# DeepLearnPhysics/dynamic-gcnn

Hardware: AMD Instinct MI355X
Metric: point-clouds/sec fwd+bwd at (B,N,k,C)=(24,2048,20,3), 1/2/4/8 MI355X (higher is better)
Workload: dtype f32

## Files before the change

### dynamic-gcnn_amd/csrc/knn.hip

```cpp
#include "knn_common.h"
#include <type_traits>
#include <stdlib.h>

namespace {

constexpr int ROWS = 64;
constexpr int WAVES = 4;
constexpr int TJ = 128;
constexpr int PERW = TJ / WAVES;

constexpr int SQ_ROWS = 64;
__global__ __launch_bounds__(256) void sqnorm_kernel(const float* __restrict__ x, int64_t ldx, int64_t rows, int C,
                                                     float* __restrict__ sq) {
  extern __shared__ float sq_tile[];
  const int64_t r0 = (int64_t)blockIdx.x * SQ_ROWS;
  const int t = threadIdx.x;
  const int S = C + 1;
  for (int e = t; e < SQ_ROWS * C; e += 256) {
    const int rr = e / C, cc = e - rr * C;
    if (r0 + rr < rows) sq_tile[rr * S + cc] = x[(r0 + rr) * ldx + cc];
  }
  __syncthreads();
  if (t < SQ_ROWS && r0 + t < rows) {
    float s = 0.0f;
// ... 1035 lines not shown
        qn = 0;
      }
    }
  }
  if (qn > 0) process(qn, 0, (nt - 1) & 1);
  __syncthreads();
  if (tid < ROWS && row0 + tid < N) cnt[grow0 + tid] = cnt_s[tid];
}

__global__ __launch_bounds__(256) void knn_select_kernel(const unsigned long long* __restrict__ ent, const int* __restrict__ cnt,
                                                         int64_t rows, int cap, int k, int32_t* __restrict__ idx) {
  const int lane = threadIdx.x & 63;
  const int64_t row = (int64_t)blockIdx.x * 4 + (threadIdx.x >> 6);
  if (row >= rows) return;
  const int S = cnt[row];
  const unsigned long long* buf = ent + row * cap;
  int32_t* out = idx + row * k;
  if (S <= 64) {
    unsigned long long key = (lane < S) ? buf[lane] : ~0ull;
    key = wave_sort64(key, lane);
    if (lane < k) out[lane] = (int32_t)(unsigned)key;
    return;
  }
  unsigned long long key[KA_MAXE];
#pragma unroll
  for (int q = 0; q < KA_MAXE; ++q) {
    const int e = lane + 64 * q;
    key[q] = (e < S) ? buf[e] : ~0ull;
  }
  const unsigned long long best = wave_lowest64<KA_MAXE>(key, S, lane);
  if (lane < k) out[lane] = (int32_t)(unsigned)best;
}

int g_knn_bf16f = -1;
int knn_bf16f_mode() {
  if (g_knn_bf16f < 0) {
    const char* e = getenv("DGCNN_KNN_BF16F");
    g_knn_bf16f = e ? ((e[0] == 'a') ? 2 : atoi(e)) : 2;
  }
  return g_knn_bf16f;
}

int g_knn_valu = 0;
bool knn_force_valu() { return g_knn_valu == 1; }

template <int LP, int MAXSTEPS, class Clouds = DenseClouds>
__global__ __launch_bounds__(256) void knn_seed_bound_kernel(const float* __restrict__ x, const float* __restrict__ sq, Clouds cl,
                                                             int64_t ldx, const int32_t* __restrict__ seed, int64_t ldseed, int k,
                                                             int64_t rows, float* __restrict__ tau0) {
  constexpr int PPS = 64 / LP;
  constexpr int RW = 2;
  const int lane = threadIdx.x & 63;
  const int64_t per = ((rows + 7) / 8 + 4 * RW - 1) / (4 * RW) * (4 * RW);
  const int64_t g0 = (int64_t)(blockIdx.x & 7) * per + ((int64_t)(blockIdx.x >> 3) * 4 + (threadIdx.x >> 6)) * RW;
  if (g0 >= rows || ((int64_t)(blockIdx.x >> 3) * 4 + (threadIdx.x >> 6)) * RW >= per) return;
  const int slot = lane / LP, cq = lane % LP;
  const int steps = (k + PPS - 1) / PPS;
  int jj[RW], nn[RW];
  int64_t gr[RW];
  const float* xc[RW];
  const float* sc[RW];
#pragma unroll
  for (int w = 0; w < RW; ++w) {
    gr[w] = (g0 + w < rows) ? g0 + w : rows - 1;
    jj[w] = (lane < k) ? seed[gr[w] * ldseed + lane] : -1 - lane;
    if constexpr (Clouds::kPacked) {
// ... 118 lines not shown
int dispatch_k(const float* x, const float* sq, int B, int N, int C, int64_t ldx, int k, int vec_ok,
               int32_t* idx, const float* tau0, hipStream_t st) {
  if (k <= 8) launch_knn<CP, 8>(x, sq, B, N, C, ldx, k, vec_ok, idx, tau0, st);
  else if (k <= 20) launch_knn<CP, 20>(x, sq, B, N, C, ldx, k, vec_ok, idx, tau0, st);
  else if (k <= 40) launch_knn<CP, 40>(x, sq, B, N, C, ldx, k, vec_ok, idx, tau0, st);
  else launch_knn<CP, 64>(x, sq, B, N, C, ldx, k, vec_ok, idx, tau0, st);
  return dg::check_launch("dgcnn_knn_f32");
}

}

extern "C" int dgcnn_knn_force_valu(int on) {
  const int prev = knn_force_valu() ? 1 : 0;
  g_knn_valu = on ? 1 : 0;
  return prev;
}

extern "C" int dgcnn_knn_bf16_filter(int mode) {
  const int prev = knn_bf16f_mode();
  g_knn_bf16f = mode;
  return prev;
}

namespace dg {
size_t knn_grid_workspace_bytes(int B, int N);
bool knn_grid_applicable(int C, int k);
int knn_grid_min_n();
int launch_knn_grid(const float* x, const float* sq, int B, int N, int C, int64_t ldx, int k, int32_t* idx, void* ws, hipStream_t st);
size_t knn_grid_seg_workspace_bytes(int rows, int nseg);
int launch_knn_grid_seg(const float* x, const float* sq, int nseg, const int32_t* seg_off, int rows, int max_n, int C, int64_t ldx, int k,
                        int32_t* idx, void* ws, hipStream_t st);
}

static size_t knn_sq_bytes(int B, int N) { return (((size_t)B * (size_t)N * sizeof(float)) + 255) & ~(size_t)255; }
static bool knn_append_lx(int N) { return N < 8192; }
static int knn_append_cap(int k, int N) {
  if (knn_append_lx(N)) return k <= 20 ? 256 : (k <= 40 ? 384 : 512);
  return k <= 20 ? 320 : (k <= 40 ? 448 : 512);
}
static bool knn_append_shape(int C, int k) { return C > 16 && C <= 64 && C % 4 == 0 && k <= 64; }
static size_t knn_append_rows_bytes(size_t rows, int cap) {
  return ((rows * sizeof(int) + 255) & ~(size_t)255) + rows * (size_t)cap * sizeof(unsigned long long);
}
static size_t knn_append_bytes(int B, int N, int k) { return knn_append_rows_bytes((size_t)B * (size_t)N, knn_append_cap(k, N)); }
static int knn_append_tighten_mask(bool lx) {
  static int tight = -1;
  if (tight < 0) { const char* e = getenv("DGCNN_KNN_TIGHTEN_EVERY"); tight = e ? atoi(e) : 0; if (tight < 0 || (tight & (tight - 1))) tight = 1; }
  return (tight ? tight : (lx ? 4 : 8)) - 1;
}

extern "C" int64_t dgcnn_knn_workspace_bytes(int B, int N, int C, int k) {
  if (B <= 0 || N <= 0) return 0;
  size_t n = 2 * knn_sq_bytes(B, N);
  if (dg::knn_grid_applicable(C, k)) n += dg::knn_grid_workspace_bytes(B, N);
  else if (knn_append_shape(C, k)) n += knn_append_bytes(B, N, k);
  return (int64_t)n;
}

static int g_knn_seed_min_n = -2;
static int knn_seed_min_n() {
  if (g_knn_seed_min_n == -2) {
    const char* e = getenv("DGCNN_KNN_SEED_MIN_N");
    g_knn_seed_min_n = e ? atoi(e) : -1;
  }
  return g_knn_seed_min_n;
}
extern "C" int dgcnn_knn_seed_min_n(int n) {
  const int prev = knn_seed_min_n();
  if (n >= -1) g_knn_seed_min_n = n;
  return prev;
}

static int g_knn_append = -1;
static bool knn_append_on() {
  if (g_knn_append < 0) {
    const char* e = getenv("DGCNN_KNN_APPEND");
    g_knn_append = e ? atoi(e) : 1;
  }
  return g_knn_append != 0;
}
extern "C" int dgcnn_knn_append(int on) {
  const int prev = knn_append_on() ? 1 : 0;
  if (on >= 0) g_knn_append = on ? 1 : 0;
  return prev;
}

static int g_knn_npr[2] = {-1, -1};
static int knn_append_products(bool lx) {
  if (g_knn_npr[0] < 0) {
    int a = 1, b = 1;
    const char* e = getenv("DGCNN_KNN_APPEND_NPR");
    if (e) sscanf(e, "%d,%d", &a, &b);
    g_knn_npr[0] = (a == 3) ? 3 : 1;
    g_knn_npr[1] = (b == 3) ? 3 : 1;
  }
  return g_knn_npr[lx ? 0 : 1];
}
extern "C" int dgcnn_knn_append_products(int n) {
  const int prev = knn_append_products(true);
  if (n == 1 || n == 3) g_knn_npr[0] = g_knn_npr[1] = n;
  return prev;
}

static int g_knn_hist = -1;
static int knn_hist_stride(int N) {
  if (g_knn_hist < 0) {
    const char* e = getenv("DGCNN_KNN_HIST");
    g_knn_hist = e ? atoi(e) : 2;
    if (g_knn_hist != 0 && g_knn_hist != 1 && g_knn_hist != 2 && g_knn_hist != 4) g_knn_hist = 2;
  }
  return N >= 256 ? g_knn_hist : 0;
}
extern "C" int dgcnn_knn_hist(int stride) {
  const int prev = knn_hist_stride(1 << 20);
  if (stride == 0 || stride == 1 || stride == 2 || stride == 4) g_knn_hist = stride;
  return prev;
}

static int knn_impl(const char* what, const float* x, int B, int N, int C, int64_t ldx, int k, const int32_t* seed, int64_t ldseed,
                    int kseed, int32_t* idx, void* ws, size_t ws_bytes, void* stream) {
  DG_REQUIRE(x && idx && ws, DGCNN_EINVAL, "%s: null pointer", what);
  DG_REQUIRE(B > 0 && N > 0 && C > 0 && ldx >= C, DGCNN_EINVAL, "%s: bad shape B=%d N=%d C=%d", what, B, N, C);
  DG_REQUIRE(k > 0 && k <= N, DGCNN_EINVAL, "%s: k=%d must be in [1, N=%d] (tf.nn.top_k raises otherwise)", what, k, N);
  DG_REQUIRE(k <= 64, DGCNN_EUNSUP, "%s: k=%d > 64 unsupported", what, k);
  DG_REQUIRE(C <= 128, DGCNN_EUNSUP, "%s: C=%d > 128 unsupported", what, C);
  DG_REQUIRE((reinterpret_cast<uintptr_t>(ws) & 15) == 0 && ws_bytes >= knn_sq_bytes(B, N), DGCNN_EINVAL,
             "%s: workspace must be 16-byte aligned and hold dgcnn_knn_workspace_bytes(B, N, C, k) bytes (got %zu)", what, ws_bytes);
  hipStream_t st = (hipStream_t)stream;
  float* sq_ws = reinterpret_cast<float*>(ws);
  const int64_t rows = (int64_t)B * N;
  const int vec_ok = (ldx % 4 == 0) && ((reinterpret_cast<uintptr_t>(x) & 15) == 0);
  const size_t grid_off = 2 * knn_sq_bytes(B, N);
  const bool append = knn_append_on() && knn_append_shape(C, k) && vec_ok && !knn_force_valu() && knn_bf16f_mode() != 0 &&
                      ws_bytes >= grid_off + knn_append_bytes(B, N, k);
  const int min_n = knn_seed_min_n() >= 0 ? knn_seed_min_n() : (append ? 0 : 4096);
  const bool seeded = seed && kseed >= k && kseed <= 64 && C > 4 && C <= 64 && C % 4 == 0 && vec_ok && !knn_force_valu() &&
                      N >= min_n && (int64_t)N * ldx < ((int64_t)1 << 31) && ws_bytes >= 2 * knn_sq_bytes(B, N);
  const bool grid_ws = dg::knn_grid_applicable(C, k) && !knn_force_valu() && ws_bytes >= grid_off + dg::knn_grid_workspace_bytes(B, N);
  dg::launch(sqnorm_kernel, dim3((unsigned)dg::cdiv(rows, SQ_ROWS)), dim3(256), sizeof(float) * SQ_ROWS * (C + 1), st, x,
                     ldx, rows, C, sq_ws);
  if (grid_ws && N >= dg::knn_grid_min_n())
    return dg::launch_knn_grid(x, sq_ws, B, N, C, ldx, k, idx, reinterpret_cast<char*>(ws) + grid_off, st);
  float* tau0 = nullptr;
  if (seeded) {
    tau0 = reinterpret_cast<float*>(reinterpret_cast<char*>(ws) + knn_sq_bytes(B, N));
    if (!launch_seed_bound(x, sq_ws, rows, DenseClouds(N), C, ldx, seed, ldseed, k, tau0, st)) tau0 = nullptr;
  }
  if (tau0 && append) {
    char* base = reinterpret_cast<char*>(ws) + grid_off;
    int* cnt = reinterpret_cast<int*>(base);
    unsigned long long* ent = reinterpret_cast<unsigned long long*>(base + (((size_t)rows * sizeof(int) + 255) & ~(size_t)255));
    const int cap = knn_append_cap(k, N);
    const dim3 grid((unsigned)dg::cdiv(N, ROWS), (unsigned)B);
    const int npr = knn_append_products(knn_append_lx(N));
    const int tmask = knn_append_tighten_mask(knn_append_lx(N));
#define DG_KA(LXV, NPRV) dg::launch((knn_bf16a_kernel<LXV, NPRV>), grid, dim3(256), 0, st, x, (const float*)sq_ws, N, C, ldx, k, (const float*)tau0, cap, ent, cnt, tmask)
    if (knn_append_lx(N)) { if (npr == 1) DG_KA(true, 1); else DG_KA(true, 3); }
    else { if (npr == 1) DG_KA(false, 1); else DG_KA(false, 3); }
#undef DG_KA
    dg::launch(knn_select_kernel, dim3((unsigned)dg::cdiv(rows, 4)), dim3(256), 0, st, (const unsigned long long*)ent, (const int*)cnt, rows,
               cap, k, idx);
    return dg::check_launch(what);
  }
  if (C <= 4) {
    const int hs = knn_hist_stride(N);
    if (hs > 0 && !knn_force_valu() && k <= 64 && N >= 4 * k * hs && ws_bytes >= 2 * knn_sq_bytes(B, N)) {
      float* tb = reinterpret_cast<float*>(reinterpret_cast<char*>(ws) + knn_sq_bytes(B, N));
      const dim3 hg((unsigned)dg::cdiv(N, 64), (unsigned)B);
      if (hs == 1) dg::launch(knn_hist_bound_kernel<1>, hg, dim3(256), 0, st, x, (const float*)sq_ws, N, C, ldx, k, tb);
      else if (hs == 2) dg::launch(knn_hist_bound_kernel<2>, hg, dim3(256), 0, st, x, (const float*)sq_ws, N, C, ldx, k, tb);
      else dg::launch(knn_hist_bound_kernel<4>, hg, dim3(256), 0, st, x, (const float*)sq_ws, N, C, ldx, k, tb);
      tau0 = tb;
    }
    return dispatch_k<4>(x, sq_ws, B, N, C, ldx, k, vec_ok, idx, tau0, st);
  }
  if (C <= 16) return dispatch_k<16>(x, sq_ws, B, N, C, ldx, k, vec_ok, idx, tau0, st);
  if (C <= 64) return dispatch_k<64>(x, sq_ws, B, N, C, ldx, k, vec_ok, idx, tau0, st);
  return dispatch_k<128>(x, sq_ws, B, N, C, ldx, k, vec_ok, idx, tau0, st);
}

extern "C" int dgcnn_knn_f32(const float* x, int B, int N, int C, int64_t ldx, int k, int32_t* idx,
                             void* ws, size_t ws_bytes, void* stream) {
  return knn_impl("dgcnn_knn_f32", x, B, N, C, ldx, k, nullptr, 0, 0, idx, ws, ws_bytes, stream);
}

extern "C" int dgcnn_knn_seeded_f32(const float* x, int B, int N, int C, int64_t ldx, int k, const int32_t* seed, int64_t ldseed,
                                    int kseed, int32_t* idx, void* ws, size_t ws_bytes, void* stream) {
  DG_REQUIRE(!seed || (ldseed >= kseed && kseed > 0), DGCNN_EINVAL, "dgcnn_knn_seeded_f32: bad seed shape");
  return knn_impl("dgcnn_knn_seeded_f32", x, B, N, C, ldx, k, seed, ldseed, kseed, idx, ws, ws_bytes, stream);
}

extern "C" int64_t dgcnn_knn_seg_workspace_bytes(int rows, int max_n, int C, int k) {
  if (rows <= 0 || max_n <= 0) return 0;
  size_t n = 2 * knn_sq_bytes(1, rows);
  if (knn_append_shape(C, k)) n += knn_append_rows_bytes((size_t)rows, knn_append_cap(k, max_n));
  return (int64_t)n;
}

extern "C" int dgcnn_knn_seg_f32(const float* x, int64_t ldx, int C, int k, int nseg, const int32_t* seg_off, int rows, int min_n,
                                 int max_n, const int32_t* seed, int64_t ldseed, int kseed, int32_t* idx, void* ws, size_t ws_bytes,
                                 void* stream) {
  const char* what = "dgcnn_knn_seg_f32";
  DG_REQUIRE(x && idx && ws && seg_off, DGCNN_EINVAL, "%s: null pointer", what);
  DG_REQUIRE(nseg > 0 && nseg <= 65535 && rows > 0 && C > 0 && ldx >= C, DGCNN_EINVAL, "%s: bad shape nseg=%d rows=%d C=%d", what,
             nseg, rows, C);
// ... 16 lines not shown
  const size_t aux = 2 * knn_sq_bytes(1, rows);
  const bool lx = knn_append_lx(max_n);
  const int cap = knn_append_cap(k, max_n);
  const bool append = knn_append_on() && knn_append_shape(C, k) && vec_ok && !knn_force_valu() && knn_bf16f_mode() != 0 &&
                      ws_bytes >= aux + knn_append_rows_bytes((size_t)rows, cap);
  const int seed_min = knn_seed_min_n() >= 0 ? knn_seed_min_n() : 0;
  const bool seeded = append && seed && kseed >= k && kseed <= 64 && min_n >= seed_min && (int64_t)max_n * ldx < ((int64_t)1 << 31);
  dg::launch(sqnorm_kernel, dim3((unsigned)dg::cdiv(rows, SQ_ROWS)), dim3(256), sizeof(float) * SQ_ROWS * (C + 1), st, x, ldx,
             (int64_t)rows, C, sq_ws);
  if (seeded && launch_seed_bound(x, sq_ws, (int64_t)rows, cl, C, ldx, seed, ldseed, k, tb, st)) {
    char* base = reinterpret_cast<char*>(ws) + aux;
    int* cnt = reinterpret_cast<int*>(base);
    unsigned long long* ent = reinterpret_cast<unsigned long long*>(base + (((size_t)rows * sizeof(int) + 255) & ~(size_t)255));
    const dim3 grid((unsigned)dg::cdiv(max_n, ROWS), (unsigned)nseg);
    const int npr = knn_append_products(lx);
    const int tmask = knn_append_tighten_mask(lx);
#define DG_KA(LXV, NPRV) dg::launch((knn_bf16a_kernel<LXV, NPRV, PackedClouds>), grid, dim3(256), 0, st, x, (const float*)sq_ws, cl, C, ldx, k, (const float*)tb, cap, ent, cnt, tmask)
    if (lx) { if (npr == 1) DG_KA(true, 1); else DG_KA(true, 3); }
    else { if (npr == 1) DG_KA(false, 1); else DG_KA(false, 3); }
#undef DG_KA
    dg::launch(knn_select_kernel, dim3((unsigned)dg::cdiv(rows, 4)), dim3(256), 0, st, (const unsigned long long*)ent, (const int*)cnt,
               (int64_t)rows, cap, k, idx);
    return dg::check_launch(what);
  }
  if (C <= 4) {
    const int hs = knn_hist_stride(min_n);
    const float* tau0 = nullptr;
    if (hs > 0 && !knn_force_valu() && min_n >= 4 * k * hs && tb_ok) {
      const dim3 hg((unsigned)dg::cdiv(max_n, 64), (unsigned)nseg);
      if (hs == 1) dg::launch(knn_hist_bound_kernel<1, PackedClouds>, hg, dim3(256), 0, st, x, (const float*)sq_ws, cl, C, ldx, k, tb);
      else if (hs == 2) dg::launch(knn_hist_bound_kernel<2, PackedClouds>, hg, dim3(256), 0, st, x, (const float*)sq_ws, cl, C, ldx, k, tb);
      else dg::launch(knn_hist_bound_kernel<4, PackedClouds>, hg, dim3(256), 0, st, x, (const float*)sq_ws, cl, C, ldx, k, tb);
      tau0 = tb;
    }
    return dispatch_k_packed<4>(x, sq_ws, cl, max_n, C, ldx, k, vec_ok, idx, tau0, st);
  }
  if (C <= 16) return dispatch_k_packed<16>(x, sq_ws, cl, max_n, C, ldx, k, vec_ok, idx, nullptr, st);
  if (C <= 64) return dispatch_k_packed<64>(x, sq_ws, cl, max_n, C, ldx, k, vec_ok, idx, nullptr, st);
  return dispatch_k_packed<128>(x, sq_ws, cl, max_n, C, ldx, k, vec_ok, idx, nullptr, st);
}

extern "C" int64_t dgcnn_knn_seg_grid_workspace_bytes(int rows, int nseg) {
  if (rows <= 0 || nseg <= 0) return 0;
  return (int64_t)(knn_sq_bytes(1, rows) + dg::knn_grid_seg_workspace_bytes(rows, nseg));
}

extern "C" int dgcnn_knn_seg_grid_f32(const float* x, int64_t ldx, int C, int k, int nseg, const int32_t* seg_off, int rows, int min_n,
                                      int max_n, int32_t* idx, void* ws, size_t ws_bytes, void* stream) {
  const char* what = "dgcnn_knn_seg_grid_f32";
  DG_REQUIRE(x && idx && ws && seg_off, DGCNN_EINVAL, "%s: null pointer", what);
  DG_REQUIRE(nseg > 0 && nseg <= 65535 && rows > 0 && C > 0 && ldx >= C, DGCNN_EINVAL, "%s: bad shape nseg=%d rows=%d C=%d", what,
             nseg, rows, C);
  DG_REQUIRE(C <= 4 && k <= 40, DGCNN_EINVAL, "%s: C=%d k=%d: the cell grid searches raw coordinates (C <= 4) for k <= 40", what, C, k);
  DG_REQUIRE(min_n > 0 && min_n <= max_n && max_n <= rows && (int64_t)min_n * nseg <= rows && (int64_t)max_n * nseg >= rows,
             DGCNN_EINVAL, "%s: cloud sizes min_n=%d max_n=%d do not fit %d rows in %d clouds", what, min_n, max_n, rows, nseg);
  DG_REQUIRE(k > 0 && k <= min_n, DGCNN_EINVAL, "%s: k=%d must be in [1, smallest cloud=%d] (tf.nn.top_k raises otherwise)", what, k,
             min_n);
  DG_REQUIRE((reinterpret_cast<uintptr_t>(ws) & 15) == 0 && ws_bytes >= (size_t)dgcnn_knn_seg_grid_workspace_bytes(rows, nseg),
             DGCNN_EINVAL, "%s: workspace must be 16-byte aligned and hold dgcnn_knn_seg_grid_workspace_bytes(rows, nseg) bytes (got %zu)",
             what, ws_bytes);
  hipStream_t st = (hipStream_t)stream;
  float* sq_ws = reinterpret_cast<float*>(ws);
  dg::launch(sqnorm_kernel, dim3((unsigned)dg::cdiv(rows, SQ_ROWS)), dim3(256), sizeof(float) * SQ_ROWS * (C + 1), st, x, ldx,
             (int64_t)rows, C, sq_ws);
  return dg::launch_knn_grid_seg(x, sq_ws, nseg, seg_off, rows, max_n, C, ldx, k, idx, reinterpret_cast<char*>(ws) + knn_sq_bytes(1, rows),
                                 st);
// ... 2 lines not shown
```

### dynamic-gcnn_amd/dgcnn/_engine.py

```python
from __future__ import annotations

import contextlib
import os
from collections import OrderedDict

import numpy as np
import torch

from . import _hip as H
from . import _planes as PL

BN_EPS = 1e-3
DROPOUT_KEEP = 0.7
WS_BYTES = 256 << 20
EDGE_MLP_LITERAL = False
EDGE_MATERIALIZE_Y = False
WGRAD_SIDE_STREAM = os.environ.get("DGCNN_SIDE_STREAM", "1") != "0"
EDGE_BWD_FUSED_L0 = True
FUSE_DROPOUT = True
BF16_FUSED_BWD = True
EDGE_BWD_REDUCE_POINTS = True
SIDE_STREAM_MIN_ROWS = 16384
SIDE_STREAM_LOW_PRIORITY = os.environ.get("DGCNN_SIDE_LOW_PRIORITY", "0") not in ("0", "")
SIDE_STREAM_RESERVE_CUS = int(os.environ.get("DGCNN_SIDE_RESERVE_CUS", "0"))
# ... 405 lines not shown
        self.min_n, self.max_n = int(sizes.min()), int(sizes.max())
        self._dev = None
        self._rg = None

    def check_k(self, k):
        if k <= 0 or k > self.min_n:
            raise ValueError("k_nn: k=%d must be in [1, smallest cloud=%d] (tf.nn.top_k raises otherwise)" % (k, self.min_n))

    def device(self, dev):
        if self._dev is None or self._dev.device != dev:
            self._dev = torch.from_numpy(self.host.astype(np.int32)).to(dev)
        return self._dev

    def row_group(self, dev):
        if self._rg is None or self._rg.device != dev:
            rg = np.repeat(np.arange(self.nseg, dtype=np.int32), np.diff(self.host))
            self._rg = torch.from_numpy(rg).to(dev)
        return self._rg


def knn(x2d, B, N, k, seed=None, seg=None):
    if seg is not None:
        return knn_packed(x2d, k, seg, seed=seed)
    C = x2d.shape[1]
    idx = torch.empty((B, N, k), dtype=torch.int32, device=x2d.device)
    nws = int(H.load().dgcnn_knn_workspace_bytes(B, N, C, k))
    ws = torch.empty((nws,), dtype=torch.uint8, device=x2d.device)
    Cp, kc = (4 if C <= 4 else 16 if C <= 16 else 64 if C <= 64 else 128), (8 if k <= 8 else 20 if k <= 20 else 40 if k <= 40 else 64)
    seeded = (KNN_SEED and seed is not None and seed.dim() == 3 and seed.shape[0] == B and seed.shape[1] == N and seed.shape[2] >= k
              and seed.dtype == torch.int32 and seed.is_contiguous())
    if seeded and 16 < C <= 64:
        tag = "knn_call<C%d,k%d>[sqnorm_kernel+knn_seed_bound_kernel+knn_bf16a_kernel+knn_select_kernel]" % (Cp, kc)
    elif C <= 4:
        tag = "knn_call<C%d,k%d>[%s]" % (Cp, kc, "knn_grid_*" if N >= 4096 else "sqnorm_kernel+knn_hist_bound_kernel+knn_kernel")
    else:
        tag = "knn_call<C%d,k%d>[sqnorm_kernel+%s]" % (Cp, kc, "knn_bf16f_kernel" if N >= 8192 else "knn_mfma_kernel")
    if (KNN_SEED and seed is not None and seed.dim() == 3 and seed.shape[0] == B and seed.shape[1] == N and seed.shape[2] >= k and
            seed.dtype == torch.int32 and seed.is_contiguous()):
        H.call("dgcnn_knn_seeded_f32", x2d.data_ptr(), B, N, C, H.ld2(x2d), k, seed.data_ptr(), int(seed.shape[2]), int(seed.shape[2]),
               idx.data_ptr(), ws.data_ptr(), nws, tag=tag, work=2.0 * B * N * N * C)
    else:
        H.call("dgcnn_knn_f32", x2d.data_ptr(), B, N, C, H.ld2(x2d), k, idx.data_ptr(), ws.data_ptr(), nws, tag=tag,
               work=2.0 * B * N * N * C)
    return idx


def knn_packed(x2d, k, seg, seed=None):
    R, C = x2d.shape
    if R != seg.rows:
        raise ValueError("offsets end at %d, the tower has %d rows" % (seg.rows, R))
    seg.check_k(k)
    off = seg.device(x2d.device)
    idx = torch.empty((1, R, k), dtype=torch.int32, device=x2d.device)
    n = seg.host[1:] - seg.host[:-1]
    Cp, kc = (4 if C <= 4 else 16 if C <= 16 else 64 if C <= 64 else 128), (8 if k <= 8 else 20 if k <= 20 else 40 if k <= 40 else 64)
    if C <= 4 and H.load().dgcnn_knn_seg_grid_use(C, k, seg.nseg, R, seg.min_n, seg.max_n, int((n * n).sum())):
        nws = int(H.load().dgcnn_knn_seg_grid_workspace_bytes(R, seg.nseg))
        ws = torch.empty((nws,), dtype=torch.uint8, device=x2d.device)
        H.call("dgcnn_knn_seg_grid_f32", x2d.data_ptr(), H.ld2(x2d), C, k, seg.nseg, off.data_ptr(), R, seg.min_n, seg.max_n,
               idx.data_ptr(), ws.data_ptr(), nws, tag="knn_seg_call<C4,k%d>[sqnorm_kernel+knn_grid_*]" % kc,
               work=2.0 * float((n * n).sum()) * C)
        return idx
    nws = int(H.load().dgcnn_knn_seg_workspace_bytes(R, seg.max_n, C, k))
    ws = torch.empty((nws,), dtype=torch.uint8, device=x2d.device)
    seeded = (KNN_SEED and seed is not None and seed.dim() == 3 and seed.shape[0] == 1 and seed.shape[1] == R and seed.shape[2] >= k
              and seed.dtype == torch.int32 and seed.is_contiguous())
    if seeded and 16 < C <= 64:
# ... 811 lines not shown
```

### dynamic-gcnn_amd/dgcnn/_hip.py

```python
from __future__ import annotations

import ctypes
import os

import torch

_HERE = os.path.dirname(os.path.abspath(__file__))
LIB_PATH = os.environ.get("DGCNN_HIP_LIB") or os.path.join(_HERE, "libdgcnn_hip.so")
STAT_SLOTS = 32

c_int, c_i64, c_f32, c_f64, c_vp, c_sz, c_u64 = (ctypes.c_int, ctypes.c_int64, ctypes.c_float, ctypes.c_double,
                                                  ctypes.c_void_p, ctypes.c_size_t, ctypes.c_uint64)

PROTOTYPES = {
    "dgcnn_version": [],
    "dgcnn_last_error": [],
    "dgcnn_knn_workspace_bytes": [c_int, c_int, c_int, c_int],
    "dgcnn_knn_grid": [c_int],
    "dgcnn_knn_force_valu": [c_int],
    "dgcnn_knn_bf16_filter": [c_int],
    "dgcnn_knn_f32": [c_vp, c_int, c_int, c_int, c_i64, c_int, c_vp, c_vp, c_sz, c_vp],
    "dgcnn_knn_seed_min_n": [c_int],
    "dgcnn_knn_append": [c_int],
    "dgcnn_knn_append_products": [c_int],
    "dgcnn_knn_hist": [c_int],
    "dgcnn_knn_seeded_f32": [c_vp, c_int, c_int, c_int, c_i64, c_int, c_vp, c_i64, c_int, c_vp, c_vp, c_sz, c_vp],
    "dgcnn_knn_seg_workspace_bytes": [c_int, c_int, c_int, c_int],
    "dgcnn_knn_seg_f32": [c_vp, c_i64, c_int, c_int, c_int, c_vp, c_int, c_int, c_int, c_vp, c_i64, c_int, c_vp, c_vp, c_sz, c_vp],
    "dgcnn_knn_seg_grid_workspace_bytes": [c_int, c_int],
    "dgcnn_knn_seg_grid_f32": [c_vp, c_i64, c_int, c_int, c_int, c_vp, c_int, c_int, c_int, c_vp, c_vp, c_sz, c_vp],
    "dgcnn_knn_seg_grid_use": [c_int, c_int, c_int, c_int, c_int, c_int, c_i64],
    "dgcnn_edge_gather_f32": [c_vp, c_i64, c_vp, c_int, c_int, c_int, c_int, c_vp, c_vp],
    "dgcnn_edge_gather_bwd_f32": [c_vp, c_vp, c_int, c_int, c_int, c_int, c_vp, c_i64, c_vp],
    "dgcnn_edge_mlp_f32": [c_vp, c_i64, c_vp, c_vp, c_int, c_int, c_int, c_int, c_int, c_vp, c_vp, c_vp],
    "dgcnn_edge_mlp_wgrad_f32": [c_vp, c_i64, c_vp, c_vp, c_int, c_int, c_int, c_int, c_int, c_vp, c_f32,
                                 c_vp, c_sz, c_vp],
    "dgcnn_edge_mlp_dgrad_scatter_f32": [c_vp, c_vp, c_vp, c_int, c_int, c_int, c_int, c_int, c_vp, c_i64, c_vp],
    "dgcnn_edge_nbr_gemm_f32": [c_vp, c_i64, c_vp, c_vp, c_vp, c_i64, c_int, c_int, c_int, c_int, c_int, c_vp, c_vp, c_vp],
    "dgcnn_edge_nbr_wgrad_f32": [c_vp, c_i64, c_vp, c_vp, c_int, c_int, c_int, c_int, c_int, c_vp, c_f32,
                                 c_vp, c_sz, c_vp],
    "dgcnn_edge_csr_build": [c_vp, c_int, c_int, c_int, c_vp, c_vp, c_vp, c_vp],
    "dgcnn_edge_gather_sum_f32": [c_vp, c_vp, c_vp, c_i64, c_int, c_vp, c_i64, c_vp],
    "dgcnn_edge_weight_split_f32": [c_vp, c_int, c_int, c_vp, c_vp],
    "dgcnn_edge_gather_add_f32": [c_vp, c_i64, c_vp, c_i64, c_vp, c_int, c_int, c_int, c_int, c_vp, c_vp, c_vp],
    "dgcnn_edge_wgrad_combine_f32": [c_vp, c_int, c_int, c_vp, c_vp],
    "dgcnn_edge_bn_act_kreduce_f32": [c_vp, c_i64, c_vp, c_i64, c_vp, c_int, c_int, c_int, c_int, c_vp, c_vp, c_vp,
                                      c_int, c_vp, c_i64, c_vp, c_i64, c_vp, c_vp],
    "dgcnn_edge_bn_bwd_reduce_f32": [c_vp, c_i64, c_vp, c_i64, c_vp, c_int, c_int, c_int, c_int, c_vp, c_vp, c_vp,
                                     c_int, c_vp, c_i64, c_vp, c_i64, c_vp, c_i64, c_vp, c_vp, c_vp],
    "dgcnn_edge_bn_bwd_reduce_points_f32": [c_vp, c_i64, c_vp, c_i64, c_vp, c_vp, c_i64, c_vp, c_i64, c_vp, c_i64, c_int,
                                            c_int, c_vp, c_vp],
    "dgcnn_edge_bn_bwd_apply_f32": [c_vp, c_i64, c_vp, c_i64, c_vp, c_int, c_int, c_int, c_int, c_vp, c_vp, c_vp,
                                    c_int, c_vp, c_i64, c_vp, c_i64, c_vp, c_i64, c_vp, c_vp, c_vp, c_vp, c_i64, c_vp,
                                    c_f32, c_vp],
    "dgcnn_edge_bn_bwd_apply_wgrad_f32": [c_vp, c_i64, c_vp, c_i64, c_vp, c_int, c_int, c_int, c_int, c_vp, c_vp, c_vp,
                                          c_vp, c_i64, c_vp, c_i64, c_vp, c_i64, c_vp, c_vp, c_vp, c_i64, c_int, c_vp, c_vp, c_f32,
                                          c_vp, c_sz, c_vp],
    "dgcnn_bn1_act_dropout_f32": [c_vp, c_i64, c_int, c_vp, c_vp, c_vp, c_int, c_f32, c_vp, c_vp, c_i64, c_vp],
# ... 53 lines not shown
    "dgcnn_adam_f32": [c_vp, c_vp, c_vp, c_vp, c_i64, c_f32, c_f32, c_f32, c_f32, c_vp],
    "dgcnn_edge_mlp_bf16_supported": [c_int, c_int, c_int],
    "dgcnn_round_bf16_f32": [c_vp, c_vp, c_i64, c_vp],
    "dgcnn_edge_mlp_bf16": [c_vp, c_i64, c_vp, c_vp, c_int, c_int, c_int, c_int, c_int, c_vp, c_vp],
    "dgcnn_edge_mlp_bf16_stats": [c_vp, c_i64, c_vp, c_vp, c_int, c_int, c_int, c_int, c_int, c_vp, c_vp],
    "dgcnn_edge_mlp_bf16_bn_kreduce": [c_vp, c_i64, c_vp, c_vp, c_int, c_int, c_int, c_int, c_int, c_vp, c_vp, c_vp, c_vp, c_i64,
                                       c_vp, c_i64, c_vp, c_int, c_vp],
    "dgcnn_edge_mlp_bf16_bwd_supported": [c_int, c_int, c_int],
    "dgcnn_edge_mlp_bf16_bwd_workspace_bytes": [c_int, c_int, c_int, c_int, c_int],
    "dgcnn_edge_mlp_bf16_bwd": [c_vp, c_i64, c_vp, c_vp, c_int, c_int, c_int, c_int, c_int, c_vp, c_vp, c_vp, c_vp, c_i64, c_vp,
                                c_vp, c_i64, c_vp, c_i64, c_vp, c_vp, c_vp, c_i64, c_vp, c_vp, c_f32, c_vp, ctypes.c_size_t, c_vp],
    "dgcnn_edge_gather_sum_bf16": [c_vp, c_vp, c_vp, c_i64, c_int, c_vp, c_i64, c_vp],
    "dgcnn_plan_begin": [],
    "dgcnn_plan_end": [c_vp],
    "dgcnn_plan_abort": [],
    "dgcnn_plan_replay": [c_vp],
    "dgcnn_plan_info": [c_vp, c_vp, c_vp, c_vp, c_vp],
    "dgcnn_plan_destroy": [c_vp],
    "dgcnn_stream_wait": [c_vp, c_vp],
    "dgcnn_stream_create": [c_int, c_int, c_vp],
    "dgcnn_stream_destroy": [c_vp],
    "dgcnn_stream_priority_range": [c_vp, c_vp],
    "dgcnn_memset_async": [c_vp, c_int, c_sz, c_vp],
    "dgcnn_comm_available": [],
    "dgcnn_comm_unique_id": [c_vp],
    "dgcnn_comm_init": [c_int, c_int, c_vp, c_vp],
    "dgcnn_comm_destroy": [c_vp],
    "dgcnn_comm_info": [c_vp, c_vp, c_vp, c_vp],
    "dgcnn_allreduce_f32": [c_vp, c_i64, c_vp, c_vp],
    "dgcnn_broadcast_f32": [c_vp, c_i64, c_int, c_vp, c_vp],
    "dgcnn_comm_counters": [c_vp, c_vp],
}

INT64_RESULTS = ("dgcnn_knn_workspace_bytes", "dgcnn_knn_seg_workspace_bytes", "dgcnn_knn_seg_grid_workspace_bytes",
                 "dgcnn_edge_mlp_bf16_bwd_workspace_bytes", "dgcnn_seg_colsum_workspace_bytes")

_lib = None


class HipError(RuntimeError):
    pass


def load():
    global _lib
    if _lib is None:
        if not os.path.exists(LIB_PATH):
            raise HipError("libdgcnn_hip.so not built (%s); run `python -c 'import __graft_entry__ as g; g.build()'` "
                           "or `make -C dynamic-gcnn_amd/csrc` -- there is no CPU fallback" % LIB_PATH)
        lib = ctypes.CDLL(LIB_PATH)
        for name, args in PROTOTYPES.items():
            fn = getattr(lib, name)
            fn.argtypes = args
            fn.restype = (ctypes.c_char_p if name == "dgcnn_last_error" else
                          ctypes.c_int64 if name in INT64_RESULTS else ctypes.c_int)
        _lib = lib
    return _lib


def set_gemm_arith(mode):
    lib = load()
    if lib.dgcnn_gemm_set_arith(int(mode)) != 0:
        raise ValueError(lib.dgcnn_last_error().decode())


def set_stat_slots(n):
    global STAT_SLOTS
# ... 160 lines not shown
```

### include/dgcnn_hip.h

```cpp
#ifndef DGCNN_HIP_H_
#define DGCNN_HIP_H_

#include <stddef.h>
#include <stdint.h>

#ifdef __cplusplus
extern "C" {
#endif

#define DGCNN_OK 0
#define DGCNN_EINVAL (-1)
#define DGCNN_ELAUNCH (-2)
#define DGCNN_ENOSPC (-3)
#define DGCNN_EUNSUP (-4)

#define DGCNN_STAT_SLOTS 32
int dgcnn_set_stat_slots(int n);
int dgcnn_get_stat_slots(void);

int dgcnn_version(void);
const char* dgcnn_last_error(void);

int64_t dgcnn_knn_workspace_bytes(int B, int N, int C, int k);
int dgcnn_knn_grid(int mode);
int dgcnn_knn_force_valu(int on);
int dgcnn_knn_bf16_filter(int mode);
int dgcnn_knn_f32(const float* x, int B, int N, int C, int64_t ldx, int k, int32_t* idx,
                  void* ws, size_t ws_bytes, void* stream);
int dgcnn_knn_seeded_f32(const float* x, int B, int N, int C, int64_t ldx, int k, const int32_t* seed, int64_t ldseed,
                         int kseed, int32_t* idx, void* ws, size_t ws_bytes, void* stream);
int dgcnn_knn_seed_min_n(int n);
int dgcnn_knn_append(int on);
int dgcnn_knn_append_products(int n);
int dgcnn_knn_hist(int stride);
int64_t dgcnn_knn_seg_workspace_bytes(int rows, int max_n, int C, int k);
int dgcnn_knn_seg_f32(const float* x, int64_t ldx, int C, int k, int nseg, const int32_t* seg_off, int rows, int min_n, int max_n,
                      const int32_t* seed, int64_t ldseed, int kseed, int32_t* idx, void* ws, size_t ws_bytes, void* stream);
int64_t dgcnn_knn_seg_grid_workspace_bytes(int rows, int nseg);
int dgcnn_knn_seg_grid_f32(const float* x, int64_t ldx, int C, int k, int nseg, const int32_t* seg_off, int rows, int min_n, int max_n,
                           int32_t* idx, void* ws, size_t ws_bytes, void* stream);
int dgcnn_knn_seg_grid_use(int C, int k, int nseg, int rows, int min_n, int max_n, int64_t sum_n2);

int dgcnn_edge_mlp_bf16_supported(int C, int k, int F);
int dgcnn_edge_mlp_bf16_bwd_supported(int C, int k, int F);
int64_t dgcnn_edge_mlp_bf16_bwd_workspace_bytes(int B, int N, int C, int k, int F);
int dgcnn_edge_mlp_bf16_bwd(const float* x, int64_t ldx, const int32_t* idx, const float* W0, int B, int N, int C, int k, int F,
                            const float* mean, const float* rstd, const float* beta, const float* mx, int64_t ldmx,
                            const float* cnt, const float* dmx, int64_t lddmx, const float* dmn, int64_t lddmn, double* red,
                            void* dYb, float* dysum, int64_t lddysum, float* dW0, float* dbeta, float dbeta_beta, void* ws,
                            size_t ws_bytes, void* stream);
int dgcnn_edge_gather_sum_bf16(const void* dY, const int32_t* off, const int32_t* rev, int64_t R, int F, float* S, int64_t lds,
                               void* stream);
int dgcnn_round_bf16_f32(const float* src, float* dst, int64_t n, void* stream);
int dgcnn_edge_mlp_bf16(const float* x, int64_t ldx, const int32_t* idx, const float* W0, int B, int N, int C, int k, int F,
                        float* Y, void* stream);
int dgcnn_edge_mlp_bf16_stats(const float* x, int64_t ldx, const int32_t* idx, const float* W0, int B, int N, int C, int k, int F,
                              double* stats, void* stream);
int dgcnn_edge_mlp_bf16_bn_kreduce(const float* x, int64_t ldx, const int32_t* idx, const float* W0, int B, int N, int C, int k,
                                   int F, const float* mean, const float* rstd, const float* beta, float* mx, int64_t ldmx,
                                   float* mn, int64_t ldmn, float* cnt, int pack_cnt, void* stream);

int dgcnn_edge_gather_f32(const float* x, int64_t ldx, const int32_t* idx, int B, int N, int C, int k,
                          float* E, void* stream);
int dgcnn_edge_gather_bwd_f32(const float* dE, const int32_t* idx, int B, int N, int C, int k,
                              float* dx, int64_t lddx, void* stream);

int dgcnn_edge_mlp_f32(const float* x, int64_t ldx, const int32_t* idx, const float* W0,
// ... 199 lines not shown
```

Before: 5547.

## Add raw-append KNN scan with in-kernel compaction for low-dimensional point clouds

For C<=4 with the histogram bound path, this adds a new scan kernel that appends candidates under a threshold into per-row global buffers. When a buffer nears capacity, the kernel compacts it in place with a wave-level top-k and tightens the threshold. A separate select kernel then extracts the final k. It replaces the register top-k list kernel, aiming to cut per-candidate insertion cost, at the expense of extra workspace, global-memory traffic and a second launch. The new path is on by default and gated by workspace size.

Result: no change. 5584, median of 6 (+0.7%).

```diff
diff --git a/dynamic-gcnn_amd/csrc/knn.hip b/dynamic-gcnn_amd/csrc/knn.hip
--- a/dynamic-gcnn_amd/csrc/knn.hip
+++ b/dynamic-gcnn_amd/csrc/knn.hip
@@ -1091,6 +1091,130 @@
   if (lane < k) out[lane] = (int32_t)(unsigned)best;
 }
 
+constexpr int RA_TJ = 128;
+constexpr int RA_PERW = RA_TJ / WAVES;
+static_assert(RA_PERW == 32, "one 32-bit verdict mask per lane and tile");
+
+__device__ __forceinline__ unsigned shl1_carry(unsigned v, lmask_t m) {
+  unsigned r;
+  lmask_t co;
+  asm("v_addc_co_u32_e64 %0, %1, %2, %2, %3" : "=v"(r), "=&s"(co) : "v"(v), "s"(m));
+  return r;
+}
+
+template <class Clouds = DenseClouds>
+__global__ __launch_bounds__(256) void knn_raw_append_kernel(const float* __restrict__ x, const float* __restrict__ sq, Clouds cl, int C,
+                                                             int64_t ldx, int k, const float* __restrict__ tau0, int cap, int pitch,
+                                                             unsigned long long* __restrict__ ent, int* __restrict__ cnt,
+                                                             int* __restrict__ ncomp) {
+  __shared__ float4 tile[RA_TJ];
+  __shared__ float ts[RA_TJ];
+  __shared__ float thr_s[ROWS];
+  __shared__ int cnt_s[ROWS];
+  __shared__ int ncomp_s[ROWS];
+  const int tid = threadIdx.x;
+  const int lane = tid & 63;
+  const int w = tid >> 6;
+  const int b = blockIdx.y;
+  const int N = cl.size(b);
+  if (Clouds::kPacked && (int)blockIdx.x * ROWS >= N) return;
+  const int64_t cb = cl.base(b);
+  const int row0 = blockIdx.x * ROWS;
+  const int row = row0 + lane;
+  const float* xb = x + cb * ldx;
+  const float* sqb = sq + cb;
+  const int rowc = row < N ? row : N - 1;
+  float xi[4];
+#pragma unroll
+  for (int c = 0; c < 4; ++c) xi[c] = (c < C) ? xb[(int64_t)rowc * ldx + c] : 0.0f;
+  const float si = sqb[rowc];
+  const int64_t grow0 = cb + row0;
+  unsigned long long* mybuf = ent + (grow0 + lane) * pitch;
+  const int trig = cap - RA_TJ;
+  const int jbase = Clouds::kPacked ? (int)cb : 0;
+  if (tid < ROWS) {
+    thr_s[tid] = (row < N) ? next_up(tau0[cb + row]) : -INFINITY;
+    cnt_s[tid] = 0;
+    ncomp_s[tid] = 0;
+  }
+  auto dist = [&](const float4& v, float sj) -> float {
+    float p = 0.f;
+    p = fmaf(xi[0], v.x, p);
+    p = fmaf(xi[1], v.y, p);
+    p = fmaf(xi[2], v.z, p);
+    p = fmaf(xi[3], v.w, p);
+    const float tt = si + sj;
+    const float tp = 2.0f * p;
+    return tt - tp;
+  };
+  float4 pre = make_float4(0.f, 0.f, 0.f, 0.f);
+  float pre_s = INFINITY;
+  auto fetch = [&](int j0) {
+    pre = make_float4(0.f, 0.f, 0.f, 0.f);
+    pre_s = INFINITY;
+    if (tid < RA_TJ && j0 + tid < N) {
+      const float* src = xb + (int64_t)(j0 + tid) * ldx;
+      pre = make_float4(src[0], (C > 1) ? src[1] : 0.f, (C > 2) ? src[2] : 0.f, (C > 3) ? src[3] : 0.f);
+      pre_s = sqb[j0 + tid];
+    }
+  };
+  fetch(0);
+  const float4* tw = tile + w * RA_PERW;
+  const float* sw = ts + w * RA_PERW;
+#pragma unroll 1
+  for (int j0 = 0; j0 < N; j0 += RA_TJ) {
+    __syncthreads();
+    if (tid < RA_TJ) {
+      tile[tid] = pre;
+      ts[tid] = pre_s;
+    }
+    if (j0 + RA_TJ < N) fetch(j0 + RA_TJ);
+    {
+      const bool over = lane < ROWS / WAVES && cnt_s[w + WAVES * lane] > trig;
+      unsigned long long need = __ballot(over);
+      while (need != 0ull) {
+        const int r = w + WAVES * (int)__builtin_ctzll(need);
+        need &= need - 1ull;
+        const int S = cnt_s[r];
+        unsigned long long* buf = ent + (grow0 + r) * pitch;
+        unsigned long long key[KA_MAXE];
+#pragma unroll
+        for (int q = 0; q < KA_MAXE; ++q) {
+          const int e = lane + 64 * q;
+          key[q] = (e < S) ? __hip_atomic_load(buf + e, __ATOMIC_RELAXED, __HIP_MEMORY_SCOPE_AGENT) : ~0ull;
+        }
+        const unsigned long long best = wave_lowest64<KA_MAXE>(key, S, lane);
+        if (lane < k) buf[lane] = best;
+        if (lane == k - 1) {
+          thr_s[r] = next_up(knn_key_dist(best));
+          cnt_s[r] = k;
+          ncomp_s[r] += 1;
+        }
+      }
+    }
+    __syncthreads();
+    if (j0 + w * RA_PERW >= N) continue;
+    const float thr = thr_s[lane];
+    unsigned mask = 0u;
+#pragma unroll
+    for (int g = 0; g < RA_PERW; ++g) mask = shl1_carry(mask, m_flt(dist(tw[g], sw[g]), thr));
+    while (__any(mask != 0u)) {
+      if (mask != 0u) {
+        const int g = 31 - __builtin_ctz(mask);
+        mask &= mask - 1u;
+        const float d = dist(tw[g], sw[g]);
+        const int pos = atomicAdd(&cnt_s[lane], 1);
+        if (pos < cap) mybuf[pos] = knn_key(d, jbase + j0 + w * RA_PERW + g);
+      }
+    }
+  }
+  __syncthreads();
+  if (tid < ROWS && row < N) {
+    cnt[grow0 + tid] = cnt_s[tid] < cap ? cnt_s[tid] : cap;
+    ncomp[grow0 + tid] = ncomp_s[tid];
+  }
+}
+
 int g_knn_bf16f = -1;
 int knn_bf16f_mode() {
   if (g_knn_bf16f < 0) {
@@ -1275,6 +1399,7 @@
                         int32_t* idx, void* ws, hipStream_t st);
 }
 
+static size_t knn_raw_bytes(size_t rows, int k);
 static size_t knn_sq_bytes(int B, int N) { return (((size_t)B * (size_t)N * sizeof(float)) + 255) & ~(size_t)255; }
 static bool knn_append_lx(int N) { return N < 8192; }
 static int knn_append_cap(int k, int N) {
@@ -1295,8 +1420,12 @@
 extern "C" int64_t dgcnn_knn_workspace_bytes(int B, int N, int C, int k) {
   if (B <= 0 || N <= 0) return 0;
   size_t n = 2 * knn_sq_bytes(B, N);
-  if (dg::knn_grid_applicable(C, k)) n += dg::knn_grid_workspace_bytes(B, N);
-  else if (knn_append_shape(C, k)) n += knn_append_bytes(B, N, k);
+  if (C <= 4) {
+    const size_t g = dg::knn_grid_applicable(C, k) ? dg::knn_grid_workspace_bytes(B, N) : 0;
+    const bool scan = !(dg::knn_grid_applicable(C, k) && N >= dg::knn_grid_min_n()) && k <= 64;
+    const size_t r = scan ? knn_raw_bytes((size_t)B * (size_t)N, k) : 0;
+    n += g > r ? g : r;
+  } else if (knn_append_shape(C, k)) n += knn_append_bytes(B, N, k);
   return (int64_t)n;
 }
 
@@ -1358,6 +1487,53 @@
   const int prev = knn_hist_stride(1 << 20);
   if (stride == 0 || stride == 1 || stride == 2 || stride == 4) g_knn_hist = stride;
   return prev;
+}
+
+static int knn_raw_cap(int k) { return k <= 20 ? 240 : (k <= 40 ? 368 : 496); }
+static size_t knn_raw_ints_bytes(size_t rows) { return (rows * sizeof(int) + 255) & ~(size_t)255; }
+static size_t knn_raw_bytes(size_t rows, int k) { return 2 * knn_raw_ints_bytes(rows) + rows * (size_t)knn_raw_cap(k) * sizeof(unsigned long long); }
+static int g_knn_raw_append = -1;
+static bool knn_raw_append_on() {
+  if (g_knn_raw_append < 0) {
+    const char* e = getenv("DGCNN_KNN_RAW_APPEND");
+    g_knn_raw_append = e ? (atoi(e) != 0 ? 1 : 0) : 1;
+  }
+  return g_knn_raw_append != 0;
+}
+extern "C" int dgcnn_knn_raw_append(int on) {
+  const int prev = knn_raw_append_on() ? 1 : 0;
+  if (on >= 0) g_knn_raw_append = on ? 1 : 0;
+  return prev;
+}
+static int g_knn_raw_guard = 0;
+extern "C" int dgcnn_knn_raw_append_guard(int entries) {
+  const int prev = g_knn_raw_guard;
+  if (entries >= 0 && entries <= 16) g_knn_raw_guard = entries;
+  return prev;
+}
+extern "C" int64_t dgcnn_knn_raw_append_workspace_bytes(int64_t rows, int k, int64_t* layout) {
+  if (rows <= 0 || rows > 0x7fffffffll || k <= 0 || k > 64) return 0;
+  const size_t off = 2 * ((((size_t)rows * sizeof(float)) + 255) & ~(size_t)255);
+  if (layout) {
+    layout[0] = (int64_t)off;
+    layout[1] = (int64_t)(off + knn_raw_ints_bytes((size_t)rows));
+    layout[2] = (int64_t)(off + 2 * knn_raw_ints_bytes((size_t)rows));
+    layout[3] = knn_raw_cap(k);
+  }
+  return (int64_t)(off + knn_raw_bytes((size_t)rows, k));
+}
+template <class Clouds>
+static int launch_raw_append(const char* what, const float* x, const float* sq, Clouds cl, dim3 grid, int64_t rows, int C, int64_t ldx,
+                             int k, const float* tau0, int32_t* idx, char* base, hipStream_t st) {
+  int* cnt = reinterpret_cast<int*>(base);
+  int* ncomp = reinterpret_cast<int*>(base + knn_raw_ints_bytes((size_t)rows));
+  unsigned long long* ent = reinterpret_cast<unsigned long long*>(base + 2 * knn_raw_ints_bytes((size_t)rows));
+  const int pitch = knn_raw_cap(k);
+  dg::launch((knn_raw_append_kernel<Clouds>), grid, dim3(256), 0, st, x, sq, cl, C, ldx, k, tau0, pitch - g_knn_raw_guard, pitch, ent, cnt,
+             ncomp);
+  dg::launch(knn_select_kernel, dim3((unsigned)dg::cdiv(rows, 4)), dim3(256), 0, st, (const unsigned long long*)ent, (const int*)cnt, rows,
+             pitch, k, idx);
+  return dg::check_launch(what);
 }
 
 static int knn_impl(const char* what, const float* x, int B, int N, int C, int64_t ldx, int k, const int32_t* seed, int64_t ldseed,
@@ -1414,6 +1590,8 @@
       else if (hs == 2) dg::launch(knn_hist_bound_kernel<2>, hg, dim3(256), 0, st, x, (const float*)sq_ws, N, C, ldx, k, tb);
       else dg::launch(knn_hist_bound_kernel<4>, hg, dim3(256), 0, st, x, (const float*)sq_ws, N, C, ldx, k, tb);
       tau0 = tb;
+      if (knn_raw_append_on() && ws_bytes >= grid_off + knn_raw_bytes((size_t)rows, k))
+        return launch_raw_append(what, x, sq_ws, DenseClouds(N), hg, rows, C, ldx, k, tau0, idx, reinterpret_cast<char*>(ws) + grid_off, st);
     }
     return dispatch_k<4>(x, sq_ws, B, N, C, ldx, k, vec_ok, idx, tau0, st);
   }
@@ -1496,6 +1674,8 @@
       else if (hs == 2) dg::launch(knn_hist_bound_kernel<2, PackedClouds>, hg, dim3(256), 0, st, x, (const float*)sq_ws, cl, C, ldx, k, tb);
       else dg::launch(knn_hist_bound_kernel<4, PackedClouds>, hg, dim3(256), 0, st, x, (const float*)sq_ws, cl, C, ldx, k, tb);
       tau0 = tb;
+      if (knn_raw_append_on() && ws_bytes >= aux + knn_raw_bytes((size_t)rows, k))
+        return launch_raw_append(what, x, sq_ws, cl, hg, (int64_t)rows, C, ldx, k, tau0, idx, reinterpret_cast<char*>(ws) + aux, st);
     }
     return dispatch_k_packed<4>(x, sq_ws, cl, max_n, C, ldx, k, vec_ok, idx, tau0, st);
   }
diff --git a/dynamic-gcnn_amd/dgcnn/_engine.py b/dynamic-gcnn_amd/dgcnn/_engine.py
--- a/dynamic-gcnn_amd/dgcnn/_engine.py
+++ b/dynamic-gcnn_amd/dgcnn/_engine.py
@@ -461,7 +461,8 @@
     if seeded and 16 < C <= 64:
         tag = "knn_call<C%d,k%d>[sqnorm_kernel+knn_seed_bound_kernel+knn_bf16a_kernel+knn_select_kernel]" % (Cp, kc)
     elif C <= 4:
-        tag = "knn_call<C%d,k%d>[%s]" % (Cp, kc, "knn_grid_*" if N >= 4096 else "sqnorm_kernel+knn_hist_bound_kernel+knn_kernel")
+        scan = "knn_raw_append_kernel+knn_select_kernel" if H.load().dgcnn_knn_raw_append(-1) else "knn_kernel"
+        tag = "knn_call<C%d,k%d>[%s]" % (Cp, kc, "knn_grid_*" if N >= 4096 else "sqnorm_kernel+knn_hist_bound_kernel+" + scan)
     else:
         tag = "knn_call<C%d,k%d>[sqnorm_kernel+%s]" % (Cp, kc, "knn_bf16f_kernel" if N >= 8192 else "knn_mfma_kernel")
     if (KNN_SEED and seed is not None and seed.dim() == 3 and seed.shape[0] == B and seed.shape[1] == N and seed.shape[2] >= k and
diff --git a/dynamic-gcnn_amd/dgcnn/_hip.py b/dynamic-gcnn_amd/dgcnn/_hip.py
--- a/dynamic-gcnn_amd/dgcnn/_hip.py
+++ b/dynamic-gcnn_amd/dgcnn/_hip.py
@@ -24,6 +24,9 @@
     "dgcnn_knn_append": [c_int],
     "dgcnn_knn_append_products": [c_int],
     "dgcnn_knn_hist": [c_int],
+    "dgcnn_knn_raw_append": [c_int],
+    "dgcnn_knn_raw_append_workspace_bytes": [c_i64, c_int, c_vp],
+    "dgcnn_knn_raw_append_guard": [c_int],
     "dgcnn_knn_seeded_f32": [c_vp, c_int, c_int, c_int, c_i64, c_int, c_vp, c_i64, c_int, c_vp, c_vp, c_sz, c_vp],
     "dgcnn_knn_seg_workspace_bytes": [c_int, c_int, c_int, c_int],
     "dgcnn_knn_seg_f32": [c_vp, c_i64, c_int, c_int, c_int, c_vp, c_int, c_int, c_int, c_vp, c_i64, c_int, c_vp, c_vp, c_sz, c_vp],
@@ -143,7 +146,7 @@
     "dgcnn_comm_counters": [c_vp, c_vp],
 }
 
-INT64_RESULTS = ("dgcnn_knn_workspace_bytes", "dgcnn_knn_seg_workspace_bytes", "dgcnn_knn_seg_grid_workspace_bytes",
+INT64_RESULTS = ("dgcnn_knn_workspace_bytes", "dgcnn_knn_seg_workspace_bytes", "dgcnn_knn_seg_grid_workspace_bytes", "dgcnn_knn_raw_append_workspace_bytes",
                  "dgcnn_edge_mlp_bf16_bwd_workspace_bytes", "dgcnn_seg_colsum_workspace_bytes")
 
 _lib = None
diff --git a/include/dgcnn_hip.h b/include/dgcnn_hip.h
--- a/include/dgcnn_hip.h
+++ b/include/dgcnn_hip.h
@@ -33,6 +33,9 @@
 int dgcnn_knn_append(int on);
 int dgcnn_knn_append_products(int n);
 int dgcnn_knn_hist(int stride);
+int dgcnn_knn_raw_append(int on);
+int64_t dgcnn_knn_raw_append_workspace_bytes(int64_t rows, int k, int64_t* layout);
+int dgcnn_knn_raw_append_guard(int entries);
 int64_t dgcnn_knn_seg_workspace_bytes(int rows, int max_n, int C, int k);
 int dgcnn_knn_seg_f32(const float* x, int64_t ldx, int C, int k, int nseg, const int32_t* seg_off, int rows, int min_n, int max_n,
                       const int32_t* seed, int64_t ldseed, int kseed, int32_t* idx, void* ws, size_t ws_bytes, void* stream);
diff --git a/profiles/knn_raw_append_bench.py b/profiles/knn_raw_append_bench.py
--- /dev/null
+++ b/profiles/knn_raw_append_bench.py
@@ -0,0 +1,39 @@
+import os
+import sys
+sys.path.insert(0, os.path.join(os.path.dirname(os.path.abspath(__file__)), "..", "dynamic-gcnn_amd"))
+import numpy as np
+import torch
+from dgcnn import _engine as E, _hip as H
+
+lib = H.load()
+rounds, reps = 7, 50
+rng = np.random.default_rng(0)
+for (B, N, C, k) in ((24, 2048, 3, 20), (24, 1024, 3, 20)):
+    x = torch.from_numpy(rng.random((B * N, C), dtype=np.float32)).cuda()
+    prev = lib.dgcnn_knn_raw_append(-1)
+    res = {0: [], 1: []}
+    ref = None
+    try:
+        for r in range(rounds + 1):
+            for on in (0, 1):
+                lib.dgcnn_knn_raw_append(on)
+                idx = E.knn(x, B, N, k)
+                if ref is None:
+                    ref = idx.clone()
+                assert torch.equal(idx, ref)
+                torch.cuda.synchronize()
+                a, b = torch.cuda.Event(enable_timing=True), torch.cuda.Event(enable_timing=True)
+                a.record()
+                for _ in range(reps):
+                    E.knn(x, B, N, k)
+                b.record()
+                torch.cuda.synchronize()
+                if r > 0:
+                    res[on].append(a.elapsed_time(b) * 1000.0 / reps)
+    finally:
+        lib.dgcnn_knn_raw_append(prev)
+    print("(B, N, C, k) = %s, %d rounds of %d calls, us per call (sqnorm + histogram + scan [+ selection])" % ((B, N, C, k), rounds, reps))
+    for on, name in ((0, "list kernel"), (1, "append form")):
+        v = res[on]
+        print("  %-12s %s  median %.1f  spread %.1f" % (name, " ".join("%.1f" % t for t in v), float(np.median(v)), max(v) - min(v)))
+    print("  append / list = %.3f" % (float(np.median(res[1])) / float(np.median(res[0]))))
```
